# a1exwang/raytracing_rb

Hardware: AMD Instinct MI355X
Metric: Mpixels/sec at 1920×1080, 4× AA, depth 5; per-channel RMS vs ref (higher is better)
Workload: dtype f64; 1 GPU; C2: 64 spheres + ground plane + area light (soft shadows), 1920x1080, 4x AA, depth 5; width=1920, height=1080, samples_per_pixel=4, trace_depth=5, objects=65, seed=1, engine=levels, parallelism=1 GPU

## Files before the change

### raytracing_rb_amd/csrc/rtx_device.h

```cpp
#pragma once
#include <hip/hip_runtime.h>

#include <algorithm>
#include <type_traits>

#include "rtx_launch.h"
#include "rtx_scene.h"
#include "rtx_vec3.h"

namespace rtx {

constexpr double PI = 3.141592653589793;
constexpr double EPS = 1e-5;
typedef float F2 __attribute__((ext_vector_type(2)));

struct Ray {
  V3 o, d;
};

struct Item {
  Ray ray;
  V3 att;
  uint64_t path;
  int32_t depth;
// ... 204 lines not shown

__device__ __forceinline__ XrRay xr_ray(float Sx, float dd, double radius, float qerr) {
  XrRay x;
  const float rad = (float)radius, kn = rad * __builtin_amdgcn_rsqf(dd);
  x.k = rad * __builtin_amdgcn_rcpf(dd);
  x.mb = 32.0f * 5.9604645e-8f * Sx * (1.0f + kn) + (2.0f + kn) * qerr;
  x.all = !(__builtin_isfinite(x.k) && __builtin_isfinite(x.mb) && dd > 0.0f);
  return x;
}

__device__ __forceinline__ bool xr_band(const XrRay& x, float dd, float l, float q, float sq, float R) {
  const float t = fabsf(R - x.k * fabsf(q));
  const float lo = fmaxf(t - x.mb, 0.0f), hi = t + x.mb;
  const float e = 4e-6f * (sq + hi * hi) * dd;
  return x.all || (l >= lo * lo * dd - e && l <= hi * hi * dd + e);
}

template <bool COUNT, typename SPH>
__device__ __forceinline__ void query(const SceneDev& S, SPH sph, bool ext, V3 o, V3 d,
                                      V3 L, double radius, double& best, int& besti, V3& bhit, bool& bin,
                                      double& total, uint32_t& err, unsigned long long* cnt, bool xr = false) {
  const double r = vr(d);
  const double r2 = r * r;
#ifndef RTX_LAZY_DN
#define RTX_LAZY_DN 0
#endif
  V3 dn = d;
  bool have_dn = false;
  if (!RTX_LAZY_DN) {
    if (r != 0) dn = v3(d.x / r, d.y / r, d.z / r);
// ... 147 lines not shown
    n = COVER_K - 1;
  }
  int k = n;
  while (k > 0) {
    const int pi = ci[(k - 1) * BS];
    if (pi < obj) break;
    ci[k * BS] = pi;
    cv[k * BS] = cv[(k - 1) * BS];
    k--;
  }
  ci[k * BS] = obj;
  cv[k * BS] = val;
  n++;
}

struct SlabRay {
  float ox, oy, oz, dx, dy, dz, dd, Sx, ms2, mS, kline, qneg;
  F2 pix, piy, piz, pax, pay, paz;
  bool fin;
};

__device__ __forceinline__ SlabRay slab_setup(const SceneDev& S, V3 o, V3 d) {
  SlabRay s;
  s.ox = (float)o.x, s.oy = (float)o.y, s.oz = (float)o.z;
  s.dx = (float)d.x, s.dy = (float)d.y, s.dz = (float)d.z;
  s.dd = __builtin_fmaf(s.dx, s.dx, __builtin_fmaf(s.dy, s.dy, s.dz * s.dz));
  s.Sx = fabsf(s.ox) + fabsf(s.oy) + fabsf(s.oz) + S.sph_scale;
  s.ms2 = CULL_M * s.Sx * s.Sx;
  s.mS = CULL_M * s.Sx;
  s.kline = s.dd * s.ms2;
  s.qneg = -CULL_M * s.Sx * sqrtf(s.dd);
  const float l1 = fabsf(s.dx) + fabsf(s.dy) + fabsf(s.dz);
  const float tiny = 1e-20f * l1;
  const float ex = fabsf(s.dx) < tiny ? copysignf(tiny, s.dx) : s.dx;
  const float ey = fabsf(s.dy) < tiny ? copysignf(tiny, s.dy) : s.dy;
  const float ez = fabsf(s.dz) < tiny ? copysignf(tiny, s.dz) : s.dz;
  const float ix = 1.0f / ex, iy = 1.0f / ey, iz = 1.0f / ez;
  const float ax = (s.ox + s.mS) * ix, ay = (s.oy + s.mS) * iy, az = (s.oz + s.mS) * iz;
  const float bx = (s.ox - s.mS) * ix, by = (s.oy - s.mS) * iy, bz = (s.oz - s.mS) * iz;
  s.pix = F2{ix, ix}, s.piy = F2{iy, iy}, s.piz = F2{iz, iz};
  s.pax = F2{-ax, -bx}, s.pay = F2{-ay, -by}, s.paz = F2{-az, -bz};
  s.fin = __builtin_isfinite(s.dd) && __builtin_isfinite(s.Sx) && l1 > 0.0f && __builtin_isfinite(ix) &&
          __builtin_isfinite(iy) && __builtin_isfinite(iz);
  return s;
}

template <typename NR>
// ... 94 lines not shown
__device__ __forceinline__ void leaf_records(const QLeaf& l, int v, float4& cx, float4& cy, float4& cz, float4& cw) {
  const uint4 a = l.q[(v >> 2) * 2], b = l.q[(v >> 2) * 2 + 1];
  auto lo = [](uint32_t w) { return (float)(w & 0xffffu); };
  auto hi = [](uint32_t w) { return (float)(w >> 16); };
  cx = make_float4(__builtin_fmaf(lo(a.x), l.sx, l.ox), __builtin_fmaf(hi(a.x), l.sx, l.ox),
                   __builtin_fmaf(lo(a.y), l.sx, l.ox), __builtin_fmaf(hi(a.y), l.sx, l.ox));
  cy = make_float4(__builtin_fmaf(lo(a.z), l.sy, l.oy), __builtin_fmaf(hi(a.z), l.sy, l.oy),
                   __builtin_fmaf(lo(a.w), l.sy, l.oy), __builtin_fmaf(hi(a.w), l.sy, l.oy));
  cz = make_float4(__builtin_fmaf(lo(b.x), l.sz, l.oz), __builtin_fmaf(hi(b.x), l.sz, l.oz),
                   __builtin_fmaf(lo(b.y), l.sz, l.oz), __builtin_fmaf(hi(b.y), l.sz, l.oz));
  const float r0 = lo(b.z) * l.rs, r1 = hi(b.z) * l.rs, r2 = lo(b.w) * l.rs, r3 = hi(b.w) * l.rs;
  cw = make_float4(r0 * r0, r1 * r1, r2 * r2, r3 * r3);
}

template <int BS, typename LP, typename XP, typename OP>
__device__ __forceinline__ void walk_leaf(int lf, LP leaf4, XP x64, OP xobj, const SlabRay& s, bool ext, V3 o, V3 d,
                                          V3 dn, double r, double r2, V3 L, double radius, double& best, int& besti,
                                          V3& bhit, bool& bin, float& thi, uint32_t& err, int* ci, double* cv,
                                          int& ncov, bool& ovf, bool xr, float qerr, int after = -1) {
  const int v = ~lf;
  const int slot0 = (v >> 2) * BVH_LEAF;
  const int cnt = (v & 3) + 1;
  float4 cx, cy, cz, cw;
  leaf_records(leaf4, v, cx, cy, cz, cw);
  uint32_t keep = 0, xkeep = 0;
  const XrRay xrr = xr ? xr_ray(s.Sx, s.dd, radius, qerr) : XrRay{};
  const F2 po = {s.ox, s.ox}, poy = {s.oy, s.oy}, poz = {s.oz, s.oz};
  const F2 pdx = {s.dx, s.dx}, pdy = {s.dy, s.dy}, pdz = {s.dz, s.dz}, pdd = {s.dd, s.dd};
  const F2 pkl = {s.kline, s.kline}, pms = {s.ms2, s.ms2};
#pragma unroll
  for (int h = 0; h < 2; h++) {
    const F2 X = h ? F2{cx.z, cx.w} : F2{cx.x, cx.y}, Y = h ? F2{cy.z, cy.w} : F2{cy.x, cy.y};
    const F2 Z = h ? F2{cz.z, cz.w} : F2{cz.x, cz.y}, Wr = h ? F2{cw.z, cw.w} : F2{cw.x, cw.y};
    const F2 ocx = X - po, ocy = Y - poy, ocz = Z - poz;
    const F2 sq = __builtin_elementwise_fma(ocx, ocx, __builtin_elementwise_fma(ocy, ocy, ocz * ocz));
    const F2 q = __builtin_elementwise_fma(ocx, pdx, __builtin_elementwise_fma(ocy, pdy, ocz * pdz));
    const F2 l = __builtin_elementwise_fma(sq, pdd, -(q * q));
    const F2 rr = __builtin_elementwise_fma(pdd, Wr, pkl);
    const F2 wm = Wr + pms;
    const bool m0 = l.x > rr.x || (q.x < s.qneg && sq.x > wm.x);
    const bool m1 = l.y > rr.y || (q.y < s.qneg && sq.y > wm.y);
    keep |= (m0 ? 0u : 1u << (2 * h)) | (m1 ? 0u : 2u << (2 * h));
    if (xr)
      xkeep |= (xr_band(xrr, s.dd, l.x, q.x, sq.x, __builtin_amdgcn_sqrtf(Wr.x)) ? 1u << (2 * h) : 0u) |
               (xr_band(xrr, s.dd, l.y, q.y, sq.y, __builtin_amdgcn_sqrtf(Wr.y)) ? 2u << (2 * h) : 0u);
  }
  keep &= (1u << cnt) - 1u;
  xkeep &= (1u << cnt) - 1u;
  while (xkeep && !(err & 0xffu)) {
    const int u = __builtin_ctz(xkeep);
    xkeep &= xkeep - 1;
    const Sphere64 sp64 = x64[slot0 + u];
    if (penumbra_raises(v3(sp64.c[0], sp64.c[1], sp64.c[2]), sp64.r, o, d, radius)) seterr(err, ERR_DOMAIN);
  }
  while (keep) {
    const int u = __builtin_ctz(keep);
    keep &= keep - 1;
    const Sphere64 sp64 = x64[slot0 + u];
    const V3 C = v3(sp64.c[0], sp64.c[1], sp64.c[2]);
    V3 hit;
// ... 38 lines not shown
  if (ax >= ay && ax >= az) {
    face = vx < 0.0f ? 1 : 0, m = ax, fs = vy, ft = vz;
  } else if (ay >= az) {
    face = vy < 0.0f ? 3 : 2, m = ay, fs = vz, ft = vx;
  } else {
    face = vz < 0.0f ? 5 : 4, m = az, fs = vx, ft = vy;
  }
  if (!(m > 0.0f)) return -1;
  const float h = 0.5f * (float)n / m;
  i = min(max((int)floorf(__builtin_fmaf(fs, h, 0.5f * (float)n)), 0), n - 1);
  j = min(max((int)floorf(__builtin_fmaf(ft, h, 0.5f * (float)n)), 0), n - 1);
  return (face * n + i) * n + j;
}

template <typename LP, typename XP>
__device__ __forceinline__ void leaf_raises(int lf, LP leaf4, XP x64, const SlabRay& s, const XrRay& xrr, V3 o, V3 d,
                                            double radius, uint32_t& err) {
  const int v = ~lf;
  const int slot0 = (v >> 2) * BVH_LEAF;
  const int cnt = (v & 3) + 1;
  float4 cx, cy, cz, cw;
  leaf_records(leaf4, v, cx, cy, cz, cw);
  const F2 po = {s.ox, s.ox}, poy = {s.oy, s.oy}, poz = {s.oz, s.oz};
  const F2 pdx = {s.dx, s.dx}, pdy = {s.dy, s.dy}, pdz = {s.dz, s.dz}, pdd = {s.dd, s.dd};
  uint32_t xkeep = 0;
#pragma unroll
  for (int h = 0; h < 2; h++) {
    const F2 X = h ? F2{cx.z, cx.w} : F2{cx.x, cx.y}, Y = h ? F2{cy.z, cy.w} : F2{cy.x, cy.y};
    const F2 Z = h ? F2{cz.z, cz.w} : F2{cz.x, cz.y}, Wr = h ? F2{cw.z, cw.w} : F2{cw.x, cw.y};
    const F2 ocx = X - po, ocy = Y - poy, ocz = Z - poz;
    const F2 sq = __builtin_elementwise_fma(ocx, ocx, __builtin_elementwise_fma(ocy, ocy, ocz * ocz));
    const F2 q = __builtin_elementwise_fma(ocx, pdx, __builtin_elementwise_fma(ocy, pdy, ocz * pdz));
    const F2 l = __builtin_elementwise_fma(sq, pdd, -(q * q));
    xkeep |= (xr_band(xrr, s.dd, l.x, q.x, sq.x, __builtin_amdgcn_sqrtf(Wr.x)) ? 1u << (2 * h) : 0u) |
             (xr_band(xrr, s.dd, l.y, q.y, sq.y, __builtin_amdgcn_sqrtf(Wr.y)) ? 2u << (2 * h) : 0u);
  }
  xkeep &= (1u << cnt) - 1u;
  while (xkeep && !(err & 0xffu)) {
    const int u = __builtin_ctz(xkeep);
    xkeep &= xkeep - 1;
    const Sphere64 sp64 = x64[slot0 + u];
    if (penumbra_raises(v3(sp64.c[0], sp64.c[1], sp64.c[2]), sp64.r, o, d, radius)) seterr(err, ERR_DOMAIN);
  }
}

__device__ __forceinline__ void sphere_record(const float4* l, int slot, float& cx, float& cy, float& cz, float& w) {
  const float* f = reinterpret_cast<const float*>(l + (slot >> 2) * BVH_LEAF);
  const int u = slot & 3;
  cx = f[u], cy = f[4 + u], cz = f[8 + u], w = f[12 + u];
}
__device__ __forceinline__ void sphere_record(const QLeaf& l, int slot, float& cx, float& cy, float& cz, float& w) {
  const uint32_t* q = reinterpret_cast<const uint32_t*>(l.q + (slot >> 2) * 2);
  const int u = slot & 3, sh = (u & 1) * 16, k = u >> 1;
  auto f16 = [sh](uint32_t x) { return (float)((x >> sh) & 0xffffu); };
  cx = __builtin_fmaf(f16(q[k]), l.sx, l.ox);
  cy = __builtin_fmaf(f16(q[2 + k]), l.sy, l.oy);
  cz = __builtin_fmaf(f16(q[4 + k]), l.sz, l.oz);
  const float r = f16(q[6 + k]) * l.rs;
  w = r * r;
}

template <typename LP, typename XP>
__device__ __forceinline__ void sphere_raises(int slot, LP leaf4, XP x64, const SlabRay& s, const XrRay& xrr, V3 o,
                                              V3 d, double radius, uint32_t& err) {
  float cx, cy, cz, w;
  sphere_record(leaf4, slot, cx, cy, cz, w);
  const float ocx = cx - s.ox, ocy = cy - s.oy, ocz = cz - s.oz;
  const float sq = __builtin_fmaf(ocx, ocx, __builtin_fmaf(ocy, ocy, ocz * ocz));
  const float q = __builtin_fmaf(ocx, s.dx, __builtin_fmaf(ocy, s.dy, ocz * s.dz));
  const float l = __builtin_fmaf(sq, s.dd, -(q * q));
  if (!xr_band(xrr, s.dd, l, q, sq, __builtin_amdgcn_sqrtf(w))) return;
  const Sphere64 sp64 = x64[slot];
  if (penumbra_raises(v3(sp64.c[0], sp64.c[1], sp64.c[2]), sp64.r, o, d, radius)) seterr(err, ERR_DOMAIN);
}

constexpr float QA_SLACK = 0.7f;
__device__ __forceinline__ bool raise_qa(float f2, float lf2, const SlabRay& s, float& qa) {
  qa = 8.0f * (__builtin_fmaf((float)__float_as_int(s.dd), 1.0f / 8388608.0f, -127.0f) - lf2);
  return s.dd >= f2 * (1.0f + 2.1e-4f) && qa + QA_SLACK <= 254.0f;
}
__device__ __forceinline__ float raise_rq(float lf2, const SlabRay& s) { return 8.0f * (__log2f(s.dd) - lf2); }

template <typename LP, typename XP>
__device__ __forceinline__ void raise_lists(const SceneDev& S, int light, const uint16_t* gates, LP leaf4, XP x64,
                                            const SlabRay& s, const XrRay& xrr, V3 o, V3 d, double radius, int face,
                                            int i, int j, float qa, float lf2, uint32_t& err) {
  const int nu = S.lbuf_n, nc = S.rbuf_n, cells = 6 * nc * nc;
  const float im = S.rbuf_inv_m;
  auto up = [im](int k) { return (int)(((float)k + 0.5f) * im); };
  const int pc = (face * nc + up(i)) * nc + up(j), mc = ((face ^ 1) * nc + up(nu - 1 - i)) * nc + up(nu - 1 - j);
  bool o2 = true, o1 = true, om = true;
  if (!S.rbuf_sphere) {
    const uint32_t gp = gates[8 + pc], gm = gates[8 + mc];
    const uint32_t g2 = gp & 31u, g1 = (gp >> 5) & 31u, gmm = (gm >> 10) & 31u;
    constexpr float U = (float)GATE_UNIT;
    o2 = g2 == 31u || qa <= U * (float)g2, o1 = qa + QA_SLACK >= U * (float)g1, om = gmm == 31u || qa <= U * (float)gmm;
    if (!(o2 || o1 || om)) return;
  }
  const float ql = raise_rq(lf2, s);
  const uint32_t* blk = S.rbuf + (size_t)light * S.rbuf_stride;
// ... 48 lines not shown
          e0 = v.x, e1 = v.y, e2 = v.z, e3 = v.w;
        } else {
          e0 = ent[k], e1 = k + 1 < k1 ? ent[k + 1] : 0u, e2 = k + 2 < k1 ? ent[k + 2] : 0u,
          e3 = k + 3 < k1 ? ent[k + 3] : 0u;
        }
      }
    }
  }
}

template <int BS, typename LP, typename XP, typename OP>
__device__ __forceinline__ bool query_lbuf(const SceneDev& S, const uint16_t* lb, LP leaf4, XP x64, OP xobj, int* ci,
                                           double* cv, V3 o, V3 d, V3 L, double radius, double& best, int& besti,
                                           V3& bhit, bool& bin, double& total, uint32_t& err, bool xr = false,
                                           int light = 0, const uint16_t* gates = nullptr) {
  const SlabRay s = slab_setup(S, o, d);
  if (!s.fin) return false;
  const int n = S.lbuf_n;
  int face, i, j;
  const int cell = lbuf_cell(-s.dx, -s.dy, -s.dz, n, face, i, j);
  if (cell < 0) return false;
  xr = xr && radius > 0.0;
  float qa = 0.0f;
  const RTX_CONST LightDev& LD = cptr(S.light)[light];
  const float f2 = LD.raise_f2, lf2 = LD.raise_lf2;
  if (xr && !(S.rbuf && gates && raise_qa(f2, lf2, s, qa))) return false;
  const int k0 = lb[cell], k1 = lb[cell + 1];
  const uint16_t* ent = lb + 6 * n * n + 1;
  const double r = vr(d);
  const double r2 = r * r;
  V3 dn = d;
// ... 32 lines not shown
      ovf = false;
      walk_planes_boxes<BS>(S, false, o, d, L, r, best, besti, bhit, bin, thi, ci, cv, ncov, ovf, after);
      for (int k = k0; k < k1; k++)
        walk_leaf<BS>((int)(int16_t)ent[k], leaf4, x64, xobj, s, false, o, d, dn, r, r2, L, radius, best, besti, bhit,
                      bin, thi, err, ci, cv, ncov, ovf, false, qerr, after);
    }
    return true;
  }
  walk_covers<BS>(S, o, d, L, radius, best, besti, bhit, bin, total, err, cv, ncov, ovf, xr && RTX_OVF_XR);
  return true;
}

__device__ __forceinline__ int lit_area_raises_lbuf(const SceneDev& S, int light, V3 T, V3 L, double radius) {
  if (!(radius > 0.0) || S.n_sphere == 0) return 0;
  const V3 d = vsub(L, T);
  const SlabRay s = slab_setup(S, T, d);
  if (!s.fin) return -1;
  int face, i, j;
  const int n = S.lbuf_n;
  const int cell = lbuf_cell(-s.dx, -s.dy, -s.dz, n, face, i, j);
  if (cell < 0) return -1;
  const uint16_t* gates = S.rgate + (size_t)light * S.rgate_stride;
  float qa;
  const RTX_CONST LightDev& LD = cptr(S.light)[light];
  if (!raise_qa(LD.raise_f2, LD.raise_lf2, s, qa)) return -1;
  const uint16_t* lb = S.lbuf + (size_t)light * S.lbuf_stride;
  const int k0 = lb[cell], k1 = lb[cell + 1];
  const uint16_t* ent = lb + 6 * n * n + 1;
  const float4* leaf4 = reinterpret_cast<const float4*>(S.bvh_sph32);
  const XrRay xrr = xr_ray(s.Sx, s.dd, radius, 0.0f);
  uint32_t err = 0;
// ... 223 lines not shown
    return lit_area_raises(S, reinterpret_cast<const Bvh4Node*>(lds), reinterpret_cast<const float4*>(S.bvh_sph32),
                           S.bvh_sph64, stk, BS, T, L, radius);
  if (SPH == SPH_BVH_GLOBAL)
    return lit_area_raises(S, S.bvh, reinterpret_cast<const float4*>(S.bvh_sph32), S.bvh_sph64, stk, BS, T, L,
                           radius);
  return lit_area_raises(S, nullptr, nullptr, nullptr, (int*)nullptr, 0, T, L, radius);
}

__device__ __forceinline__ Ray reflection(const Ray& ray, V3 nn, double c, V3 hit, V3 delta, uint32_t& err) {
  Ray r;
  r.d = vnorm(vadd(vsc(nn, 2.0 * c * vr(ray.d)), ray.d), err);
  r.o = vadd(hit, delta);
  return r;
}

__device__ __forceinline__ bool refraction(const Ray& ray, V3 nn, double c, V3 hit, V3 refl, double rate,
                                           Ray& out, uint32_t& err) {
  const double sin_i = sqrt(1.0 - c * c);
  const double sin_r = sin_i / rate;
  if (sin_r >= 1) return false;
  const double r = rx_asin(sin_r);
  out.d = vadd(vsc(nn, -rx_cos(r)), vsc(vnorm(vadd(refl, ray.d), err), sin_r));
  out.o = vsub(hit, vsc(nn, EPS));
  return true;
}

__device__ __forceinline__ V3 texcolor(const SceneDev& S, int tex, double hs, double vs, double uo,
                                       double vo, double uu, double vv, uint32_t& err) {
  const TexDev t = S.tex[tex];
  const double qu = (uu + uo) / hs, qv = (vv + vo) / vs;
  if (!isfinite(qu) || !isfinite(qv)) {
    seterr(err, ERR_DOMAIN);
    return v3(0.0, 0.0, 0.0);
  }
  long iu = (long)fmod(trunc(qu), (double)t.w);
  long iv = (long)fmod(trunc(qv), (double)t.h);
  if (iu < 0) iu += t.w;
  if (iv < 0) iv += t.h;
  const uint8_t* p = S.texels + t.off + ((size_t)iv * t.w + iu) * 3;
// ... 105 lines not shown
__device__ __forceinline__ void emit(Stack& st, Item& pend, bool& has, uint32_t& err, const Ray& r,
                                     V3 att, uint64_t path, int depth) {
  if (depth <= 0 || vr(att) < 0.0001) return;
  if (has) {
    if (st.n < st.maxs) st.push(pend);
    else seterr(err, ERR_DOMAIN);
  }
  pend.ray = r;
  pend.att = att;
  pend.path = path;
  pend.depth = depth;
  has = true;
}

struct LightSum { V3 lc; int nl; };
__device__ __forceinline__ LightSum light_term(const SceneDev& S, const LightDev& L, double tot, V3 hit, V3 nn, V3 lc,
                                               int nl, uint32_t& err) {
  const double area = tot > 0 ? tot : 0.0;
  if (area > 0) {
    nl++;
    const double pw = S.sse_is_two ? area * area : rx_pow(area, S.sse);
    const V3 lcol = vsc(v3p(L.color), pw / (double)S.n_light);
    const V3 ll = vnorm(vsub(v3p(L.pos), hit), err);
    double ldn = vdot(ll, nn);
    if (ldn > 1) ldn = 1.0;
    else if (ldn < 0) ldn = 0.0;
    lc = vadd(lc, vsc(lcol, ldn));
  }
  return {lc, nl};
}

__device__ __forceinline__ void sphere_uv(const SceneDev& S, const Material& m, V3 hit, double& u, double& v,
                                          double& mm2) {
  const Sphere64 sp = S.sph64[m.rec];
  const V3 vec = vsub(hit, v3p(sp.c));
  const double x0 = vdot(vec, v3p(m.gw_n)) / sp.r;
  const double y0 = vdot(vec, v3p(m.east_n)) / sp.r;
  const double z0 = vdot(vec, v3p(m.north_n)) / sp.r;
  mm2 = x0 * x0 + y0 * y0 + z0 * z0 + 2.0 * x0 + 1.0;
  const double mm = sqrt(mm2);
  u = (y0 / mm + 1.0) / 2.0;
  v = (-z0 / mm + 1.0) / 2.0;
}

__device__ __forceinline__ V3 leaf_color(const SceneDev& S, const Material& m, V3 hit, V3 lc, int nl, uint32_t& err) {
  lc = vdiv(lc, (double)nl);
  V3 color;
  if (m.type == OBJ_BOX) {
    color = vadd(vmul(lc, v3p(m.diffuse)), v3p(m.ambient));
  } else {
    V3 filter = v3(1.0, 1.0, 1.0);
    if (m.tex >= 0) {
      if (m.type == OBJ_SPHERE) {
        double u, v, mm2;
        sphere_uv(S, m, hit, u, v, mm2);
        if (mm2 < 0) seterr(err, ERR_DOMAIN);
        filter = vmul(texcolor(S, m.tex, m.hs, m.vs, m.u_off, m.v_off, u, v, err), filter);
      } else {
        double u, v;
        plane_uv(S.planes + (size_t)m.rec * PLANE_GEO, hit, u, v);
        filter = vmul(texcolor(S, m.tex, m.hs, m.vs, 0.0, 0.0, u, v, err), filter);
// ... 27 lines not shown
  bool has = false;
  const uint64_t R = (uint64_t)cam.pt + 3;
  const double c = vcos(cur.ray.d, n, err);
  const Ray refl = reflection(cur.ray, nn, c, hit, delta, err);
  emit(st, pend, has, err, refl, vmul(cur.att, v3p(m.refl_att)), cur.path * R + 1, cur.depth - 1);
  Ray refr;
  bool has_refr = false;
  if (m.type == OBJ_SPHERE)
    has_refr = refraction(cur.ray, nn, c, hit, refl.d, in ? m.rr : 1.0 / m.rr, refr, err);
  else if (m.has_rr)
    has_refr = refraction(cur.ray, nn, c, hit, refl.d, m.rr, refr, err);
  if (has_refr)
    emit(st, pend, has, err, refr, vmul(cur.att, v3p(m.refr_att)), cur.path * R + 2, cur.depth - 1);
  if (nl == 0) {
    const int pt = cam.pt;
    const V3 att = vmul(cur.att, vdiv(v3p(m.diffuse), (double)pt));
    V3 left, up;
    pt_basis(n, nn, left, up, err);
    Ray r;
    r.o = vadd(hit, delta);
    for (int k = 0; k < pt; k++) {
      r.d = pt_dir(seed, x, y, sample, cur.path, k, nn, left, up);
      emit(st, pend, has, err, r, att, cur.path * R + 3 + (uint64_t)k, cur.depth - 1);
    }
  } else {
    add_leaf(sum, vmul(cur.att, leaf_color(S, m, hit, lc, nl, err)), err);
  }
  if (has) cur = pend;
  return has;
}

// ... 50 lines not shown
      if (c < -1) c = -1;
      fire = rx_acos(c) < L.hl_angle_rad;
    }
    if (fire) {
      fired |= 1u << l;
      nfired++;
      if (RTX_HL_RAISES && !(err & 0xffu) && raises(it.ray.o, v3(L.pos[0], L.pos[1], L.pos[2]), L.radius, l))
        seterr(err, ERR_DOMAIN);
    }
  }
  if (!nfired) return false;
  it.att = att_fn();
  for (int l = 0; l < S.n_light; l++) {
    if (!(fired >> l & 1)) continue;
    const RTX_CONST LightDev& L = lights[l];
    leaf(vdiv(vmul(it.att, vsc(v3(L.color[0], L.color[1], L.color[2]), L.hl_rate)), (double)nfired));
  }
  return true;
}

template <typename Leaf, typename Rz>
__device__ __forceinline__ bool highlight_leaves(const SceneDev& S, const Item& it, Leaf&& leaf, uint32_t& err,
                                                 Rz&& raises) {
  return highlight_leaves_att(S, it.ray, [&] { return it.att; }, leaf, err, raises);
}

template <bool REDUCE = true, typename Rz>
__device__ __forceinline__ bool highlights(const SceneDev& S, const Item& it, V3& sum, uint32_t& err, Rz&& raises) {
  return highlight_leaves(S, it, [&](V3 c) {
    if (REDUCE) add_leaf(sum, c, err);
    else sum = vadd(sum, c);
// ... 7 lines not shown
__device__ __forceinline__ unsigned long long px_key(int x, int y, int H, int phase = 0) {
  return ((unsigned long long)x * (unsigned long long)H + (unsigned long long)y) << 1 | (unsigned long long)phase;
}

__device__ __forceinline__ int row_to_y(const KParams& p, int row) {
  if (p.tile_rows == 0) return p.y0 + row;
  const int k = row / p.tile_rows;
  const int t = p.row_tiles ? p.row_tiles[k] : k * p.nranks + p.rank;
  return t * p.tile_rows + (row - k * p.tile_rows);
}

struct ItemPos {
  int px, row, sample;
  bool valid;
};
__device__ __forceinline__ ItemPos decode_item(const KParams& p, int k) {
  ItemPos ip;
  if (p.lv_pass == 0) {
    const int tiles_x = (p.nx + 7) >> 3;
    const int per = 64 * p.pre;
    const int slot = k / per, r = k - slot * per;
    const int tile = p.lv_t0 + slot * p.lv_tstride;
    const int l = r / p.pre;
    ip.sample = r - l * p.pre;
    ip.px = (tile % tiles_x) * 8 + ((l & 1) | ((l >> 1) & 2) | ((l >> 2) & 4));
    ip.row = (tile / tiles_x) * 8 + (((l >> 1) & 1) | ((l >> 2) & 2) | ((l >> 3) & 4));
    ip.valid = ip.px < p.nx && ip.row < p.nrows && row_to_y(p, ip.row) < p.cam->height;
  } else {
    const int n_extra = p.max_samples - p.pre;
    const int e = k / n_extra;
    const int idx = p.extra_list[p.lv_e0 + e];
    ip.sample = p.pre + (k - e * n_extra);
    ip.px = idx % p.nx;
    ip.row = idx / p.nx;
    ip.valid = true;
  }
  return ip;
}

// ... 51 lines not shown
```

### raytracing_rb_amd/csrc/rtx_levels.hip

```cpp
#include <vector>

#include "rtx_device.h"

namespace rtx {

constexpr int RAY_DOUBLES = 12;
constexpr int RAY_DOUBLES_SMALL = 10;
constexpr int HIT_DOUBLES = 8;
static_assert(RAY_DOUBLES * 8 == (int)RAY_BYTES && HIT_DOUBLES * 8 == (int)LV_HIT_BYTES, "record sizes");

static __device__ unsigned long long rtx_stamps_lv[8 * 8];

static __device__ unsigned long long rtx_stamps_wg[8 * 8];

#if RTX_STAMPS
static __shared__ unsigned long long lv_wg[3];
#endif
struct LvWgStamps {
  unsigned long long w0 = 0;
  __device__ __forceinline__ void begin() {
#if RTX_STAMPS
    if (threadIdx.x == 0) {
      lv_wg[0] = ~0ull;
      lv_wg[1] = 0ull;
// ... 444 lines not shown
                           reinterpret_cast<const Sphere64*>(lds + p.lds_x64),
                           reinterpret_cast<const int32_t*>(lds + p.lds_xobj), stk, cov_i, cov_v, ext, o, d, L, rad,
                           best, besti, hit, hin, total, err, q_ref, q_sp, q_ncov, q_ovf, false, 0, xr);
    else if (SPH == SPH_BVH_MIX)
      query_bvh<BS, false>(S, reinterpret_cast<const Bvh4Node*>(lds), reinterpret_cast<const float4*>(S.bvh_sph32),
                           S.bvh_sph64, S.bvh_obj, stk, cov_i, cov_v, ext, o, d, L, rad, best, besti, hit, hin, total,
                           err, q_ref, q_sp, q_ncov, q_ovf, false, 0, xr);
    else
      query_bvh<BS, false>(S, S.bvh, reinterpret_cast<const float4*>(S.bvh_sph32), S.bvh_sph64, S.bvh_obj, stk, cov_i,
                           cov_v, ext, o, d, L, rad, best, besti, hit, hin, total, err, q_ref, q_sp, q_ncov, q_ovf,
                           false, 0, xr);
  }
  return true;
}

__device__ __forceinline__ void lv_ray(const KParams& p, int level, uint32_t idx, Item& cur, int& root, int& x, int& y,
                                       int& sample, bool& valid) {
  valid = true;
  if (level == 0) {
    root = (int)idx;
    const ItemPos ip = decode_item(p, root);
    x = p.x0 + ip.px;
    y = row_to_y(p, ip.row);
    sample = ip.sample;
    valid = ip.valid;
    if (valid) {
      const CameraDev& cam = *p.cam;
      cur.ray = lens_ray(cam, lens_target(cam, x, y), x, y, sample, p.seed);
      cur.att = v3(1.0, 1.0, 1.0);
      cur.path = 1;
    }
    return;
  }
  const double2* q = reinterpret_cast<const double2*>(lv_src(p, level) + (size_t)idx * p.lv_ray_dbl);
  double2 e;
  lv_unpack_ray(q, cur.ray.o, cur.ray.d);
// ... 15 lines not shown
  char* rec;
  uint32_t errA, errL;
  int nleaf, besti;
  V3 hit;
  bool hin, ext, shade;
};

template <int SPH, int BS>
__device__ __forceinline__ void lv_first_half(const KParams& p, char* lds, int level, uint32_t slot, uint32_t i,
                                              uint32_t base, int depth, bool& active, LvFirst& f, LvStamps* st) {
  const SceneDev& S = p.scene;
  f.root = f.x = f.y = f.sample = 0;
  bool alive = false;
  if (active) {
    bool valid;
    lv_ray(p, level, slot, f.cur, f.root, f.x, f.y, f.sample, valid);
    if (level == 0) p.lv_redo_of[i] = -1;
    active = valid;
    alive = valid && (level > 0 || !(depth <= 0 || vr(f.cur.att) < 0.0001));
    if (active && base + i >= p.lv_lcap) {
      lv_redo(p, f.root);
      active = alive = false;
    }
  }
  f.rec = p.lv_rec + (size_t)(base + i) * p.lv_rec_bytes;
  double* leafp = reinterpret_cast<double*>(f.rec + 8);

  f.errA = f.errL = 0;
  f.nleaf = 0;
  bool fired = false, hl_defer = false;
  if (alive)
// ... 65 lines not shown
}

__device__ __forceinline__ void lv_finish(const KParams& p, int level, int slice, bool shade, bool active,
                                          const Item& cur, int root, int x, int y, int sample, int besti, bool hin,
                                          V3 hit, V3 delta, V3 nrm, V3 nn, double c, V3 lc, int nl, char* rec,
                                          int nleaf, uint32_t errA, uint32_t errS, uint32_t errL, uint32_t errP,
                                          const Material* m, bool last = false, bool keys = false) {
  const SceneDev& S = p.scene;
  const CameraDev& cam = *p.cam;
  const int depth = last ? 1 : cam.depth - level;
  const int pt = cam.pt;
  const uint64_t R = (uint64_t)pt + 3;
  uint32_t mask = 0;
  double rate = 0.0;
  bool may_refract = false;
  if (shade) {
    const int cd = depth - 1;
    if (cd > 0 && !(vr(vmul(cur.att, v3p(m->refl_att))) < 0.0001)) mask |= 1u;
    if (m->type == OBJ_SPHERE) {
      may_refract = true;
      rate = hin ? m->rr : 1.0 / m->rr;
    } else if (m->has_rr) {
      may_refract = true;
      rate = m->rr;
    }
    if (may_refract && !(sqrt(1.0 - c * c) / rate >= 1) && cd > 0 &&
        !(vr(vmul(cur.att, v3p(m->refr_att))) < 0.0001))
      mask |= 2u;
    if (nl == 0 && cd > 0 && !(vr(vmul(cur.att, vdiv(v3p(m->diffuse), (double)pt))) < 0.0001))
      mask |= ((1u << pt) - 1u) << 2;
  }
  const uint32_t log2cap = (uint32_t)p.lv_slice_log2, cap = 1u << log2cap;
  const int nch = __popc(mask);
  const int incl = (int)wave_scan_incl((uint32_t)nch);
  const int wtotal = __shfl(incl, 63);
  uint32_t wraw = 0;
  if (wtotal > 0 && __lane_id() == 0) wraw = atomicAdd(lv_slice_ctr(p.lv_ctl->sc[level + 1], slice), (uint32_t)wtotal);
  Ray refl, refr;
  bool has_refr = false;
  if (shade) {
    const bool refr_live = (mask & 2u) != 0;
    const bool refr_chk = may_refract && !refr_live && !(sqrt(1.0 - c * c) / rate >= 1);
    if ((mask & 1u) || refr_live || refr_chk) {
      refl = reflection(cur.ray, nn, c, hit, delta, errS);
    } else if (vr(vadd(vsc(nn, 2.0 * c * vr(cur.ray.d)), cur.ray.d)) == 0) {
      if (!errS) errS = ERR_ZERO_VEC;
    }
    if (refr_live) {
      has_refr = refraction(cur.ray, nn, c, hit, refl.d, rate, refr, errS);
    } else if (refr_chk && vr(vadd(refl.d, cur.ray.d)) == 0) {
      if (!errS) errS = ERR_ZERO_VEC;
    }
    if (nl != 0) {
      const V3 leaf = vmul(cur.att, leaf_color(S, *m, hit, lc, nl, errP));
      double* leafp = reinterpret_cast<double*>(rec + 8);
      leafp[0] = leaf.x;
      leafp[1] = leaf.y;
      leafp[2] = leaf.z;
      nleaf = 1;
    }
  }
  const uint32_t off0 = (wtotal > 0 ? (uint32_t)__shfl((int)wraw, 0) : 0u) + (uint32_t)(incl - nch);
  const uint32_t child0 = ((uint32_t)slice << log2cap) + off0;
  if (shade) {
// ... 1 lines not shown
    uint32_t off = off0;
    auto put = [&](const Ray& r, V3 att, uint64_t path) {
      if (off < cap) {
        const uint32_t at = ((uint32_t)slice << log2cap) + off;
        lv_store_ray(p, outs + (size_t)at * p.lv_ray_dbl, r, att, path, root, x, y, sample);
        if (keys) p.lv_key[at] = (uint16_t)lv_ray_bin(S, r, p.lv_cell_bits);
      } else {
        lv_redo(p, root);
        atomicAdd(&p.lv_ctl->dropped, 1u);
      }
      off++;
    };
    if (mask & 1u) put(refl, vmul(cur.att, v3p(m->refl_att)), cur.path * R + 1);
    if (has_refr) put(refr, vmul(cur.att, v3p(m->refr_att)), cur.path * R + 2);
    if (nl == 0 && (mask >> 2) != 0) {
      const V3 att = vmul(cur.att, vdiv(v3p(m->diffuse), (double)pt));
      V3 left, up;
      pt_basis(nrm, nn, left, up, errP);
      Ray r;
      r.o = vadd(hit, delta);
      lv_ray_key(p, root, x, y, sample);
      for (int k = 0; k < pt; k++) {
        r.d = pt_dir(p.seed, x, y, sample, cur.path, k, nn, left, up);
        if (mask >> (2 + k) & 1u) put(r, att, cur.path * R + 3 + (uint64_t)k);
      }
    }
  }
  if (active) {
    uint32_t err = errA;
    if (!err) err = errS;
    if (!err) err = errL;
// ... 83 lines not shown
  while (true) {
    {
      uint32_t chunk = 0;
      if (got) got = sched.claim(p, nch, chunk);
      st.begin_chunk(got);
      if (got) {
        uint32_t slot, i;
        bool active = lv_chunk_item(p, in, level, chunk, slot, i);
        const double2* qs = reinterpret_cast<const double2*>(lv_src(p, level) + (size_t)slot * p.lv_ray_dbl);
        Item cur;
        int root = 0, x = 0, y = 0, sample = 0;
        bool alive = false;
        if (active) {
          bool valid = true;
          if (level == 0) {
            lv_ray(p, level, slot, cur, root, x, y, sample, valid);
            p.lv_redo_of[i] = -1;
          } else {
            const double2 a = qs[0], b = qs[1], c = qs[2];
            cur.ray.o = v3(a.x, a.y, b.x);
            cur.ray.d = v3(b.y, c.x, c.y);
          }
          active = valid;
          alive = valid && (level > 0 || !(depth <= 0 || vr(cur.att) < 0.0001));
          if (active && base + i >= p.lv_lcap) {
            lv_redo(p, level == 0 ? root : lv_ray_root(p, qs));
            active = alive = false;
          }
        }
        char* rec = p.lv_rec + (size_t)(base + i) * p.lv_rec_bytes;
        double* leafp = reinterpret_cast<double*>(rec + 8);
// ... 119 lines not shown
    int nl = 0;
    for (int li = 0; li < S.n_light; li++) {
      if (!shade) continue;
      const LightDev& L = S.light[li];
      const V3 qL = v3p(L.pos);
      double tot = 1.0;
      double b2 = 0.0;
      int bi2 = -1;
      V3 h2 = qo;
      bool in2 = true;
      lv_walk<SPH, BS>(p, lds, false, qo, vsub(qL, qo), qL, L.radius, b2, bi2, h2, in2, tot, errL, XR, li);
      const double area = tot > 0 ? tot : 0.0;
      if (area > 0) {
        nl++;
        const double pw = S.sse_is_two ? area * area : rx_pow(area, S.sse);
        const V3 lcol = vsc(v3p(L.color), pw / (double)S.n_light);
        const V3 ll = vnorm(vsub(v3p(L.pos), hit), errP);
        double ldn = vdot(ll, nn);
        if (ldn > 1) ldn = 1.0;
        else if (ldn < 0) ldn = 0.0;
        lc = vadd(lc, vsc(lcol, ldn));
      }
    }
    st.mark(3);
    lv_finish(p, level, slice, shade, shade, cur, root, x, y, sample, besti, hin, hit, delta, nrm, nn, c, lc, nl, rec, 0,
              errA, errS, errL, errP, m, LAST, SORT);
    st.mark(5);
  }
  wgs.end(level);
  st.flush(level);
}
// ... 280 lines not shown
  if (threadIdx.x == 0) trays = 0;
  lv_layout(p, nlev, base, pex);
  const unsigned long long ts1 = RTX_STAMPS ? stamp() : 0ull;
  const int pre = p.pre;
  uint32_t* lo = lds_fin + nlev * 64 + threadIdx.x;
  uint32_t* hi = lo + SD * 256;
  double* scol = reinterpret_cast<double*>(lds_fin + nlev * 64 + (SD > 16 ? 0 : 2 * SD * 256));
  uint32_t* serr = reinterpret_cast<uint32_t*>(scol + 64 * pre * 3);
  uint32_t lo_p[SD > 16 ? LV_MAXL : 1], hi_p[SD > 16 ? LV_MAXL : 1];
  const int n_items = 64 * pre;
  const int n_tiles = p.lv_fin_tiles > (int)gridDim.x ? p.lv_fin_tiles : (int)gridDim.x;
  for (int slot = blockIdx.x; slot < n_tiles; slot += gridDim.x) {
    const int item0 = slot * n_items;
    uint32_t nvis = 0;
    for (int it = (int)threadIdx.x; it < n_items; it += 256) {
      const ItemPos ip = decode_item(p, item0 + it);
      if (!ip.valid) continue;
      uint32_t e = 0;
      const V3 c = SD > 16 ? lv_sample(p, base, pex, item0 + it, nlev, lo_p, hi_p, 1, LV_MAXL, e, nvis)
                           : lv_sample(p, base, pex, item0 + it, nlev, lo, hi, 256, SD, e, nvis);
      scol[3 * it] = c.x;
      scol[3 * it + 1] = c.y;
      scol[3 * it + 2] = c.z;
      serr[it] = e;
    }
    if (p.tile_rays) atomicAdd(&trays, nvis);
    __syncthreads();
    if (p.tile_rays && threadIdx.x == 0) {
      p.tile_rays[p.lv_t0 + slot * p.lv_tstride] = trays;
      trays = 0;
    }
// ... 613 lines not shown
```

### raytracing_rb_amd/csrc/rtx_query.hip

```cpp
#include "rtx_device.h"

namespace rtx {

constexpr int LA_BS = 256;

__device__ __forceinline__ int32_t la_status(uint32_t code) { return code == ERR_TYPE ? 8 : (int32_t)code; }

template <int SPH>
__global__ __launch_bounds__(LA_BS) void k_lit_area(KParams p, const double* __restrict__ targets,
                                                     const double* __restrict__ lights, double* __restrict__ area,
                                                     double* __restrict__ color, int32_t* __restrict__ status) {
  const SceneDev& S = p.scene;
  extern __shared__ float4 lds_la[];
  char* lds = reinterpret_cast<char*>(lds_la);
  if (SPH == SPH_BVH_LDS) {
    const int nn = S.n_nodes * (int)(sizeof(Bvh4Node) / 16);
    for (int i = threadIdx.x; i < nn; i += LA_BS) lds_la[i] = reinterpret_cast<const float4*>(S.bvh)[i];
    float4* leaf = reinterpret_cast<float4*>(lds + p.lds_leaf);
    for (int i = threadIdx.x; i < S.n_slots; i += LA_BS) leaf[i] = reinterpret_cast<const float4*>(S.bvh_sph32)[i];
    __syncthreads();
  }
  const size_t i = (size_t)blockIdx.x * LA_BS + threadIdx.x;
  if (i >= (size_t)p.nrays) return;
  int* stk = reinterpret_cast<int*>(lds + p.lds_stack) + threadIdx.x;
// ... 36 lines not shown
                                  reinterpret_cast<const float4*>(lds + p.lds_leaf), S.bvh_sph64, S.bvh_obj, stk,
                                  cov_i, cov_v, false, T, d, L, rad, best, besti, hit, hin, total, err, q_ref, q_sp,
                                  q_ncov, q_ovf, false, 0, xr);
        else
          query_bvh<LA_BS, false>(S, S.bvh, reinterpret_cast<const float4*>(S.bvh_sph32), S.bvh_sph64, S.bvh_obj,
                                  stk, cov_i, cov_v, false, T, d, L, rad, best, besti, hit, hin, total, err, q_ref,
                                  q_sp, q_ncov, q_ovf, false, 0, xr);
      }
      if (err & 0xffu) {
        st = la_status(err & 0xffu);
      } else {
        a = total > 0 ? total : 0.0;
        c = v3(0.0, 0.0, 0.0);
        if (a > 0 && color) {
          const double pw = S.sse_is_two ? a * a : rx_pow(a, S.sse);
          c = vsc(lcol, pw / (double)S.n_light);
        }
      }
    }
    const size_t o = i * (size_t)nl + (size_t)k;
    area[o] = a;
    if (color) {
      color[3 * o] = c.x;
      color[3 * o + 1] = c.y;
      color[3 * o + 2] = c.z;
    }
  }
  if (status) status[i] = st;
}

template <int SPH>
// ... 41 lines not shown
```

### raytracing_rb_amd/csrc/rtx_rtmap.hip

```cpp
#include "rtx_device.h"

namespace rtx {

constexpr int RM_BS = 256;

__device__ __forceinline__ int32_t rm_status(uint32_t code) { return code == ERR_TYPE ? 8 : (int32_t)code; }

__device__ __forceinline__ void rm_store3(double* g, V3 a) {
  if ((reinterpret_cast<uintptr_t>(g) & 15) == 0) {
    *reinterpret_cast<double2*>(g) = make_double2(a.x, a.y);
    g[2] = a.z;
  } else {
    g[0] = a.x;
    *reinterpret_cast<double2*>(g + 1) = make_double2(a.y, a.z);
  }
}
__device__ __forceinline__ void rm_store6(double* g, V3 a, V3 b) {
  if ((reinterpret_cast<uintptr_t>(g) & 15) == 0) {
    double2* g2 = reinterpret_cast<double2*>(g);
    g2[0] = make_double2(a.x, a.y);
    g2[1] = make_double2(a.z, b.x);
    g2[2] = make_double2(b.y, b.z);
  } else {
    double2* g2 = reinterpret_cast<double2*>(g + 1);
// ... 154 lines not shown
                                    q_sp, q_ncov, q_ovf, false, 0, xr);
        }
        ls = light_term(S, LD, tot, hit, nn, ls.lc, ls.nl, errP);
      }
      const Ray refl = reflection(cur.ray, nn, c, hit, delta, errS);
      put(refl, vmul(cur.att, v3p(m.refl_att)), cur.path * R + 1);
      Ray refr;
      bool has_refr = false;
      if (m.type == OBJ_SPHERE)
        has_refr = refraction(cur.ray, nn, c, hit, refl.d, hin ? m.rr : 1.0 / m.rr, refr, errS);
      else if (m.has_rr)
        has_refr = refraction(cur.ray, nn, c, hit, refl.d, m.rr, refr, errS);
      if (has_refr) put(refr, vmul(cur.att, v3p(m.refr_att)), cur.path * R + 2);
      if (ls.nl == 0) {
        kind = 4;
        const V3 a = vmul(cur.att, vdiv(v3p(m.diffuse), (double)pt));
        V3 left, up;
        pt_basis(n, nn, left, up, errP);
        Ray r;
        r.o = T;
        for (int k = 0; k < pt; k++) {
          r.d = pt_dir(p.seed, x, y, sample, cur.path, k, nn, left, up);
          put(r, a, cur.path * R + 3 + (uint64_t)k);
        }
      } else {
        kind = 3;
        const V3 leaf = vmul(cur.att, leaf_color(S, m, hit, ls.lc, ls.nl, errP));
        if (lf) rm_store3(lf, leaf);
        nleaf = 1;
      }
    }
// ... 89 lines not shown
```

Baseline: 499.1 Mpixels/s.

## Pack band test, slim leaf ray setup, skip unit divides, simplify item decode

Several micro-optimizations land together. The two-lane band test is now evaluated with packed float2 math. Light-buffer walks use a lighter ray setup that drops the slab reciprocals. Double-precision divides by light or sample counts are skipped when the count is one. The refraction sine is computed once and reused, and item decoding uses shifts for power-of-two sample counts with a wave-uniform slot. Together these cut ALU and fp64 divide work in hot paths, but small numeric differences are possible, for example in the changed finiteness check for leaf walks.

```diff
diff --git a/raytracing_rb_amd/csrc/rtx_device.h b/raytracing_rb_amd/csrc/rtx_device.h
--- a/raytracing_rb_amd/csrc/rtx_device.h
+++ b/raytracing_rb_amd/csrc/rtx_device.h
@@ -242,6 +242,18 @@
   const float lo = fmaxf(t - x.mb, 0.0f), hi = t + x.mb;
   const float e = 4e-6f * (sq + hi * hi) * dd;
   return x.all || (l >= lo * lo * dd - e && l <= hi * hi * dd + e);
+}
+
+__device__ __forceinline__ uint32_t xr_band2(const XrRay& x, float dd, F2 l, F2 q, F2 sq, F2 W) {
+  const F2 R = {__builtin_amdgcn_sqrtf(W.x), __builtin_amdgcn_sqrtf(W.y)};
+  const F2 pk = {x.k, x.k}, pmb = {x.mb, x.mb}, pdd = {dd, dd}, p4 = {4e-6f, 4e-6f};
+  const F2 d = R - pk * F2{fabsf(q.x), fabsf(q.y)};
+  const F2 t = {fabsf(d.x), fabsf(d.y)};
+  const F2 tm = t - pmb, hi = t + pmb;
+  const F2 lo = {fmaxf(tm.x, 0.0f), fmaxf(tm.y, 0.0f)};
+  const F2 e = p4 * (sq + hi * hi) * pdd;
+  const F2 a = lo * lo * pdd - e, b = hi * hi * pdd + e;
+  return ((x.all || (l.x >= a.x && l.x <= b.x)) ? 1u : 0u) | ((x.all || (l.y >= a.y && l.y <= b.y)) ? 2u : 0u);
 }
 
 template <bool COUNT, typename SPH>
@@ -419,14 +431,15 @@
   n++;
 }
 
-struct SlabRay {
+struct WalkRay {
   float ox, oy, oz, dx, dy, dz, dd, Sx, ms2, mS, kline, qneg;
-  F2 pix, piy, piz, pax, pay, paz;
   bool fin;
 };
-
-__device__ __forceinline__ SlabRay slab_setup(const SceneDev& S, V3 o, V3 d) {
-  SlabRay s;
+struct SlabRay : WalkRay {
+  F2 pix, piy, piz, pax, pay, paz;
+};
+
+__device__ __forceinline__ float walk_setup(const SceneDev& S, V3 o, V3 d, WalkRay& s) {
   s.ox = (float)o.x, s.oy = (float)o.y, s.oz = (float)o.z;
   s.dx = (float)d.x, s.dy = (float)d.y, s.dz = (float)d.z;
   s.dd = __builtin_fmaf(s.dx, s.dx, __builtin_fmaf(s.dy, s.dy, s.dz * s.dz));
@@ -435,7 +448,19 @@
   s.mS = CULL_M * s.Sx;
   s.kline = s.dd * s.ms2;
   s.qneg = -CULL_M * s.Sx * sqrtf(s.dd);
-  const float l1 = fabsf(s.dx) + fabsf(s.dy) + fabsf(s.dz);
+  return fabsf(s.dx) + fabsf(s.dy) + fabsf(s.dz);
+}
+
+__device__ __forceinline__ WalkRay leaf_setup(const SceneDev& S, V3 o, V3 d) {
+  WalkRay s;
+  const float l1 = walk_setup(S, o, d, s);
+  s.fin = __builtin_isfinite(s.dd) && __builtin_isfinite(s.Sx) && l1 >= 2e-17f;
+  return s;
+}
+
+__device__ __forceinline__ SlabRay slab_setup(const SceneDev& S, V3 o, V3 d) {
+  SlabRay s;
+  const float l1 = walk_setup(S, o, d, s);
   const float tiny = 1e-20f * l1;
   const float ex = fabsf(s.dx) < tiny ? copysignf(tiny, s.dx) : s.dx;
   const float ey = fabsf(s.dy) < tiny ? copysignf(tiny, s.dy) : s.dy;
@@ -560,7 +585,7 @@
 }
 
 template <int BS, typename LP, typename XP, typename OP>
-__device__ __forceinline__ void walk_leaf(int lf, LP leaf4, XP x64, OP xobj, const SlabRay& s, bool ext, V3 o, V3 d,
+__device__ __forceinline__ void walk_leaf(int lf, LP leaf4, XP x64, OP xobj, const WalkRay& s, bool ext, V3 o, V3 d,
                                           V3 dn, double r, double r2, V3 L, double radius, double& best, int& besti,
                                           V3& bhit, bool& bin, float& thi, uint32_t& err, int* ci, double* cv,
                                           int& ncov, bool& ovf, bool xr, float qerr, int after = -1) {
@@ -587,9 +612,7 @@
     const bool m0 = l.x > rr.x || (q.x < s.qneg && sq.x > wm.x);
     const bool m1 = l.y > rr.y || (q.y < s.qneg && sq.y > wm.y);
     keep |= (m0 ? 0u : 1u << (2 * h)) | (m1 ? 0u : 2u << (2 * h));
-    if (xr)
-      xkeep |= (xr_band(xrr, s.dd, l.x, q.x, sq.x, __builtin_amdgcn_sqrtf(Wr.x)) ? 1u << (2 * h) : 0u) |
-               (xr_band(xrr, s.dd, l.y, q.y, sq.y, __builtin_amdgcn_sqrtf(Wr.y)) ? 2u << (2 * h) : 0u);
+    if (xr) xkeep |= xr_band2(xrr, s.dd, l, q, sq, Wr) << (2 * h);
   }
   keep &= (1u << cnt) - 1u;
   xkeep &= (1u << cnt) - 1u;
@@ -658,7 +681,7 @@
 }
 
 template <typename LP, typename XP>
-__device__ __forceinline__ void leaf_raises(int lf, LP leaf4, XP x64, const SlabRay& s, const XrRay& xrr, V3 o, V3 d,
+__device__ __forceinline__ void leaf_raises(int lf, LP leaf4, XP x64, const WalkRay& s, const XrRay& xrr, V3 o, V3 d,
                                             double radius, uint32_t& err) {
   const int v = ~lf;
   const int slot0 = (v >> 2) * BVH_LEAF;
@@ -676,8 +699,7 @@
     const F2 sq = __builtin_elementwise_fma(ocx, ocx, __builtin_elementwise_fma(ocy, ocy, ocz * ocz));
     const F2 q = __builtin_elementwise_fma(ocx, pdx, __builtin_elementwise_fma(ocy, pdy, ocz * pdz));
     const F2 l = __builtin_elementwise_fma(sq, pdd, -(q * q));
-    xkeep |= (xr_band(xrr, s.dd, l.x, q.x, sq.x, __builtin_amdgcn_sqrtf(Wr.x)) ? 1u << (2 * h) : 0u) |
-             (xr_band(xrr, s.dd, l.y, q.y, sq.y, __builtin_amdgcn_sqrtf(Wr.y)) ? 2u << (2 * h) : 0u);
+    xkeep |= xr_band2(xrr, s.dd, l, q, sq, Wr) << (2 * h);
   }
   xkeep &= (1u << cnt) - 1u;
   while (xkeep && !(err & 0xffu)) {
@@ -705,7 +727,7 @@
 }
 
 template <typename LP, typename XP>
-__device__ __forceinline__ void sphere_raises(int slot, LP leaf4, XP x64, const SlabRay& s, const XrRay& xrr, V3 o,
+__device__ __forceinline__ void sphere_raises(int slot, LP leaf4, XP x64, const WalkRay& s, const XrRay& xrr, V3 o,
                                               V3 d, double radius, uint32_t& err) {
   float cx, cy, cz, w;
   sphere_record(leaf4, slot, cx, cy, cz, w);
@@ -719,15 +741,15 @@
 }
 
 constexpr float QA_SLACK = 0.7f;
-__device__ __forceinline__ bool raise_qa(float f2, float lf2, const SlabRay& s, float& qa) {
+__device__ __forceinline__ bool raise_qa(float f2, float lf2, const WalkRay& s, float& qa) {
   qa = 8.0f * (__builtin_fmaf((float)__float_as_int(s.dd), 1.0f / 8388608.0f, -127.0f) - lf2);
   return s.dd >= f2 * (1.0f + 2.1e-4f) && qa + QA_SLACK <= 254.0f;
 }
-__device__ __forceinline__ float raise_rq(float lf2, const SlabRay& s) { return 8.0f * (__log2f(s.dd) - lf2); }
+__device__ __forceinline__ float raise_rq(float lf2, const WalkRay& s) { return 8.0f * (__log2f(s.dd) - lf2); }
 
 template <typename LP, typename XP>
 __device__ __forceinline__ void raise_lists(const SceneDev& S, int light, const uint16_t* gates, LP leaf4, XP x64,
-                                            const SlabRay& s, const XrRay& xrr, V3 o, V3 d, double radius, int face,
+                                            const WalkRay& s, const XrRay& xrr, V3 o, V3 d, double radius, int face,
                                             int i, int j, float qa, float lf2, uint32_t& err) {
   const int nu = S.lbuf_n, nc = S.rbuf_n, cells = 6 * nc * nc;
   const float im = S.rbuf_inv_m;
@@ -806,7 +828,7 @@
                                            double* cv, V3 o, V3 d, V3 L, double radius, double& best, int& besti,
                                            V3& bhit, bool& bin, double& total, uint32_t& err, bool xr = false,
                                            int light = 0, const uint16_t* gates = nullptr) {
-  const SlabRay s = slab_setup(S, o, d);
+  const WalkRay s = leaf_setup(S, o, d);
   if (!s.fin) return false;
   const int n = S.lbuf_n;
   int face, i, j;
@@ -869,7 +891,7 @@
 __device__ __forceinline__ int lit_area_raises_lbuf(const SceneDev& S, int light, V3 T, V3 L, double radius) {
   if (!(radius > 0.0) || S.n_sphere == 0) return 0;
   const V3 d = vsub(L, T);
-  const SlabRay s = slab_setup(S, T, d);
+  const WalkRay s = leaf_setup(S, T, d);
   if (!s.fin) return -1;
   int face, i, j;
   const int n = S.lbuf_n;
@@ -1123,15 +1145,21 @@
   return r;
 }
 
-__device__ __forceinline__ bool refraction(const Ray& ray, V3 nn, double c, V3 hit, V3 refl, double rate,
-                                           Ray& out, uint32_t& err) {
+__device__ __forceinline__ double refract_sin(double c, double rate) {
   const double sin_i = sqrt(1.0 - c * c);
-  const double sin_r = sin_i / rate;
+  return sin_i / rate;
+}
+__device__ __forceinline__ bool refraction_sin(const Ray& ray, V3 nn, double sin_r, V3 hit, V3 refl, Ray& out,
+                                               uint32_t& err) {
   if (sin_r >= 1) return false;
   const double r = rx_asin(sin_r);
   out.d = vadd(vsc(nn, -rx_cos(r)), vsc(vnorm(vadd(refl, ray.d), err), sin_r));
   out.o = vsub(hit, vsc(nn, EPS));
   return true;
+}
+__device__ __forceinline__ bool refraction(const Ray& ray, V3 nn, double c, V3 hit, V3 refl, double rate,
+                                           Ray& out, uint32_t& err) {
+  return refraction_sin(ray, nn, refract_sin(c, rate), hit, refl, out, err);
 }
 
 __device__ __forceinline__ V3 texcolor(const SceneDev& S, int tex, double hs, double vs, double uo,
@@ -1267,13 +1295,26 @@
 }
 
 struct LightSum { V3 lc; int nl; };
+__device__ __forceinline__ double div_count(double x, int n) {
+  if (n != 1) x = x / (double)n;
+  return x;
+}
+__device__ __forceinline__ V3 vdiv_count(V3 a, int n) {
+  if (n != 1) a = vdiv(a, (double)n);
+  return a;
+}
+__device__ __forceinline__ double light_share(const SceneDev& S, double pw) { return div_count(pw, S.n_light); }
+__device__ __forceinline__ V3 vdiv_lights(const SceneDev& S, V3 a, int k) {
+  if (S.n_light == 1) return a;
+  return vdiv(a, (double)k);
+}
 __device__ __forceinline__ LightSum light_term(const SceneDev& S, const LightDev& L, double tot, V3 hit, V3 nn, V3 lc,
                                                int nl, uint32_t& err) {
   const double area = tot > 0 ? tot : 0.0;
   if (area > 0) {
     nl++;
     const double pw = S.sse_is_two ? area * area : rx_pow(area, S.sse);
-    const V3 lcol = vsc(v3p(L.color), pw / (double)S.n_light);
+    const V3 lcol = vsc(v3p(L.color), light_share(S, pw));
     const V3 ll = vnorm(vsub(v3p(L.pos), hit), err);
     double ldn = vdot(ll, nn);
     if (ldn > 1) ldn = 1.0;
@@ -1297,7 +1338,7 @@
 }
 
 __device__ __forceinline__ V3 leaf_color(const SceneDev& S, const Material& m, V3 hit, V3 lc, int nl, uint32_t& err) {
-  lc = vdiv(lc, (double)nl);
+  lc = vdiv_lights(S, lc, nl);
   V3 color;
   if (m.type == OBJ_BOX) {
     color = vadd(vmul(lc, v3p(m.diffuse)), v3p(m.ambient));
@@ -1355,7 +1396,7 @@
     emit(st, pend, has, err, refr, vmul(cur.att, v3p(m.refr_att)), cur.path * R + 2, cur.depth - 1);
   if (nl == 0) {
     const int pt = cam.pt;
-    const V3 att = vmul(cur.att, vdiv(v3p(m.diffuse), (double)pt));
+    const V3 att = vmul(cur.att, vdiv_count(v3p(m.diffuse), pt));
     V3 left, up;
     pt_basis(n, nn, left, up, err);
     Ray r;
@@ -1436,7 +1477,7 @@
   for (int l = 0; l < S.n_light; l++) {
     if (!(fired >> l & 1)) continue;
     const RTX_CONST LightDev& L = lights[l];
-    leaf(vdiv(vmul(it.att, vsc(v3(L.color[0], L.color[1], L.color[2]), L.hl_rate)), (double)nfired));
+    leaf(vdiv_lights(S, vmul(it.att, vsc(v3(L.color[0], L.color[1], L.color[2]), L.hl_rate)), nfired));
   }
   return true;
 }
@@ -1474,15 +1515,25 @@
   int px, row, sample;
   bool valid;
 };
+template <bool CHUNK = false>
 __device__ __forceinline__ ItemPos decode_item(const KParams& p, int k) {
   ItemPos ip;
   if (p.lv_pass == 0) {
     const int tiles_x = (p.nx + 7) >> 3;
-    const int per = 64 * p.pre;
-    const int slot = k / per, r = k - slot * per;
+    const int pre = p.pre, per = 64 * pre;
+    const int kb = CHUNK ? __builtin_amdgcn_readfirstlane(k) & ~63 : k;
+    int slot, l;
+    if ((pre & (pre - 1)) == 0) {
+      const int lp = 31 - __builtin_clz(pre);
+      slot = kb >> (6 + lp);
+      l = (k - slot * per) >> lp;
+    } else {
+      slot = kb / per;
+      l = (k - slot * per) / pre;
+    }
+    const int r = k - slot * per;
     const int tile = p.lv_t0 + slot * p.lv_tstride;
-    const int l = r / p.pre;
-    ip.sample = r - l * p.pre;
+    ip.sample = r - l * pre;
     ip.px = (tile % tiles_x) * 8 + ((l & 1) | ((l >> 1) & 2) | ((l >> 2) & 4));
     ip.row = (tile / tiles_x) * 8 + (((l >> 1) & 1) | ((l >> 2) & 2) | ((l >> 3) & 4));
     ip.valid = ip.px < p.nx && ip.row < p.nrows && row_to_y(p, ip.row) < p.cam->height;
diff --git a/raytracing_rb_amd/csrc/rtx_levels.hip b/raytracing_rb_amd/csrc/rtx_levels.hip
--- a/raytracing_rb_amd/csrc/rtx_levels.hip
+++ b/raytracing_rb_amd/csrc/rtx_levels.hip
@@ -482,12 +482,13 @@
   return true;
 }
 
+template <bool CHUNK = false>
 __device__ __forceinline__ void lv_ray(const KParams& p, int level, uint32_t idx, Item& cur, int& root, int& x, int& y,
                                        int& sample, bool& valid) {
   valid = true;
   if (level == 0) {
     root = (int)idx;
-    const ItemPos ip = decode_item(p, root);
+    const ItemPos ip = decode_item<CHUNK>(p, root);
     x = p.x0 + ip.px;
     y = row_to_y(p, ip.row);
     sample = ip.sample;
@@ -533,7 +534,7 @@
   bool alive = false;
   if (active) {
     bool valid;
-    lv_ray(p, level, slot, f.cur, f.root, f.x, f.y, f.sample, valid);
+    lv_ray<true>(p, level, slot, f.cur, f.root, f.x, f.y, f.sample, valid);
     if (level == 0) p.lv_redo_of[i] = -1;
     active = valid;
     alive = valid && (level > 0 || !(depth <= 0 || vr(f.cur.att) < 0.0001));
@@ -629,6 +630,8 @@
   uint32_t mask = 0;
   double rate = 0.0;
   bool may_refract = false;
+  double sin_r = 0.0;
+  bool tir = false;
   if (shade) {
     const int cd = depth - 1;
     if (cd > 0 && !(vr(vmul(cur.att, v3p(m->refl_att))) < 0.0001)) mask |= 1u;
@@ -639,10 +642,13 @@
       may_refract = true;
       rate = m->rr;
     }
-    if (may_refract && !(sqrt(1.0 - c * c) / rate >= 1) && cd > 0 &&
-        !(vr(vmul(cur.att, v3p(m->refr_att))) < 0.0001))
+    if (may_refract) {
+      sin_r = refract_sin(c, rate);
+      tir = sin_r >= 1;
+    }
+    if (may_refract && !tir && cd > 0 && !(vr(vmul(cur.att, v3p(m->refr_att))) < 0.0001))
       mask |= 2u;
-    if (nl == 0 && cd > 0 && !(vr(vmul(cur.att, vdiv(v3p(m->diffuse), (double)pt))) < 0.0001))
+    if (nl == 0 && cd > 0 && !(vr(vmul(cur.att, vdiv_count(v3p(m->diffuse), pt))) < 0.0001))
       mask |= ((1u << pt) - 1u) << 2;
   }
   const uint32_t log2cap = (uint32_t)p.lv_slice_log2, cap = 1u << log2cap;
@@ -655,14 +661,14 @@
   bool has_refr = false;
   if (shade) {
     const bool refr_live = (mask & 2u) != 0;
-    const bool refr_chk = may_refract && !refr_live && !(sqrt(1.0 - c * c) / rate >= 1);
+    const bool refr_chk = may_refract && !refr_live && !tir;
     if ((mask & 1u) || refr_live || refr_chk) {
       refl = reflection(cur.ray, nn, c, hit, delta, errS);
     } else if (vr(vadd(vsc(nn, 2.0 * c * vr(cur.ray.d)), cur.ray.d)) == 0) {
       if (!errS) errS = ERR_ZERO_VEC;
     }
     if (refr_live) {
-      has_refr = refraction(cur.ray, nn, c, hit, refl.d, rate, refr, errS);
+      has_refr = refraction_sin(cur.ray, nn, sin_r, hit, refl.d, refr, errS);
     } else if (refr_chk && vr(vadd(refl.d, cur.ray.d)) == 0) {
       if (!errS) errS = ERR_ZERO_VEC;
     }
@@ -694,7 +700,7 @@
     if (mask & 1u) put(refl, vmul(cur.att, v3p(m->refl_att)), cur.path * R + 1);
     if (has_refr) put(refr, vmul(cur.att, v3p(m->refr_att)), cur.path * R + 2);
     if (nl == 0 && (mask >> 2) != 0) {
-      const V3 att = vmul(cur.att, vdiv(v3p(m->diffuse), (double)pt));
+      const V3 att = vmul(cur.att, vdiv_count(v3p(m->diffuse), pt));
       V3 left, up;
       pt_basis(nrm, nn, left, up, errP);
       Ray r;
@@ -808,7 +814,7 @@
         if (active) {
           bool valid = true;
           if (level == 0) {
-            lv_ray(p, level, slot, cur, root, x, y, sample, valid);
+            lv_ray<true>(p, level, slot, cur, root, x, y, sample, valid);
             p.lv_redo_of[i] = -1;
           } else {
             const double2 a = qs[0], b = qs[1], c = qs[2];
@@ -958,7 +964,7 @@
       if (area > 0) {
         nl++;
         const double pw = S.sse_is_two ? area * area : rx_pow(area, S.sse);
-        const V3 lcol = vsc(v3p(L.color), pw / (double)S.n_light);
+        const V3 lcol = vsc(v3p(L.color), light_share(S, pw));
         const V3 ll = vnorm(vsub(v3p(L.pos), hit), errP);
         double ldn = vdot(ll, nn);
         if (ldn > 1) ldn = 1.0;
@@ -1269,7 +1275,7 @@
     const int item0 = slot * n_items;
     uint32_t nvis = 0;
     for (int it = (int)threadIdx.x; it < n_items; it += 256) {
-      const ItemPos ip = decode_item(p, item0 + it);
+      const ItemPos ip = decode_item<true>(p, item0 + it);
       if (!ip.valid) continue;
       uint32_t e = 0;
       const V3 c = SD > 16 ? lv_sample(p, base, pex, item0 + it, nlev, lo_p, hi_p, 1, LV_MAXL, e, nvis)
diff --git a/raytracing_rb_amd/csrc/rtx_query.hip b/raytracing_rb_amd/csrc/rtx_query.hip
--- a/raytracing_rb_amd/csrc/rtx_query.hip
+++ b/raytracing_rb_amd/csrc/rtx_query.hip
@@ -74,7 +74,7 @@
         c = v3(0.0, 0.0, 0.0);
         if (a > 0 && color) {
           const double pw = S.sse_is_two ? a * a : rx_pow(a, S.sse);
-          c = vsc(lcol, pw / (double)S.n_light);
+          c = vsc(lcol, light_share(S, pw));
         }
       }
     }
diff --git a/raytracing_rb_amd/csrc/rtx_rtmap.hip b/raytracing_rb_amd/csrc/rtx_rtmap.hip
--- a/raytracing_rb_amd/csrc/rtx_rtmap.hip
+++ b/raytracing_rb_amd/csrc/rtx_rtmap.hip
@@ -192,7 +192,7 @@
       if (has_refr) put(refr, vmul(cur.att, v3p(m.refr_att)), cur.path * R + 2);
       if (ls.nl == 0) {
         kind = 4;
-        const V3 a = vmul(cur.att, vdiv(v3p(m.diffuse), (double)pt));
+        const V3 a = vmul(cur.att, vdiv_count(v3p(m.diffuse), pt));
         V3 left, up;
         pt_basis(n, nn, left, up, errP);
         Ray r;
```

New measurement: 506.5 Mpixels/s, median of 6. +1.5%, better.
